# GarciaLnk/LlamaRec

Measured on AMD Instinct MI355X. Metric: users/sec through retrieve+rerank, higher is better.
Workload: dtype bf16; 1 GPU; beauty two-stage: LRURec(V=12086, L=50, D=64, 2 blocks) top-50 with history mask -> Llama-2-7b (32 layers, bf16, random init) single prefill -> verbalizer over 20 candidates; batching=token budget 32768 per step (llamarec_amd/packing.py), rmsnorm_folded_into_gemm=False, llama_layers=32, parallelism=dp1, collective_backend=nccl

## Files before the change

include/llamarec_mi355x.h:

```cpp
#ifndef LLAMAREC_MI355X_H
#define LLAMAREC_MI355X_H

#include <stddef.h>
#include <stdint.h>

#ifdef __cplusplus
extern "C" {
#endif

#define LR_OK 0
#define LR_EINVAL (-1)
#define LR_EUNSUPPORTED (-2)
#define LR_EHIP (-3)
#define LR_EWORKSPACE (-4)

#define LR_MAX_LRU_BLOCKS 4
#define LR_MAX_TOPK 64

const char* lr_last_error(void);
const char* lr_version(void);


typedef struct LrLruBlockWeights {
  const float* params_log;
// ... 110 lines not shown
typedef struct LrRopeScaling {
  int32_t kind;
  float factor, low_freq_factor, high_freq_factor;
  int32_t original_max_positions;
  int32_t reserved[3];
} LrRopeScaling;
int lr_llama_set_rope_scaling(lr_llama_t* h, const LrRopeScaling* s);

typedef struct LrGemma2Ext {
  float attn_softcap;
  float final_softcap;
  float attn_scale;
  int32_t reserved[5];
  const uint16_t* const* attn_out_norm;
  const uint16_t* const* mlp_out_norm;
} LrGemma2Ext;
int lr_llama_set_gemma2(lr_llama_t* h, const LrGemma2Ext* ext);

int lr_llama_set_qkv_bias(lr_llama_t* h, const uint16_t* const* bqkv);

int lr_fold_norm_bf16(const uint16_t* w, const uint16_t* norm_w, int32_t rows, int32_t cols, uint16_t* out,
                      void* hip_stream);
int lr_llama_set_folded_norms(lr_llama_t* h, const uint16_t* const* wqkv_folded, const uint16_t* const* wgu_folded);

int lr_llama_set_last_layer_pruning(lr_llama_t* h, int32_t enable);

size_t lr_llama_workspace_bytes(const lr_llama_t* h, int32_t max_tokens, int32_t max_seqs);

int lr_llama_prefill_verbalize(lr_llama_t* h, const int32_t* packed_ids, const int32_t* cu_seqlens,
                               const int32_t* cu_seqlens_host, int32_t B,
                               const int32_t* label_token_ids, int32_t C, float* out_scores,
                               void* workspace, size_t workspace_bytes, void* hip_stream);

int lr_llama_prefill_verbalize_prefix(lr_llama_t* h, const int32_t* packed_ids, const int32_t* cu_seqlens,
                                      const int32_t* cu_seqlens_host, int32_t B, int32_t prefix_len,
                                      const int32_t* label_token_ids, int32_t C, float* out_scores,
                                      void* workspace, size_t workspace_bytes, void* hip_stream);
int32_t lr_common_prefix_len(const int32_t* packed_ids_host, const int32_t* cu_seqlens_host, int32_t B);

int lr_llama_last_logits(lr_llama_t* h, const int32_t* packed_ids, const int32_t* cu_seqlens,
                         const int32_t* cu_seqlens_host, int32_t B, float* out_logits,
                         void* workspace, size_t workspace_bytes, void* hip_stream);

int lr_llama_pack_qkv(const uint16_t* q, const uint16_t* k, const uint16_t* v, int32_t num_heads,
                      int32_t num_kv_heads, int32_t head_dim, int32_t hidden, uint16_t* out);

// ... 174 lines not shown
```

llamarec_amd/_lib.py:

```python
from __future__ import annotations

import ctypes as C
import os

from . import _abi as A

_HERE = os.path.dirname(os.path.abspath(__file__))
LIB_PATH = os.environ.get("LLAMAREC_LIB") or os.path.join(_HERE, "lib", "libllamarec_mi355x.so")
_lib = None


class LlamaRecError(RuntimeError):
    pass


PROTOTYPES = {
    "lr_last_error": (C.c_char_p, []),
    "lr_version": (C.c_char_p, []),
    "lr_lru_packed_bytes": (C.c_size_t, [C.c_int32, C.c_int32]),
    "lr_lru_pack": (C.c_int, [C.POINTER(A.LrLruWeightsDesc), C.c_void_p, C.c_size_t]),
    "lr_lru_create": (C.c_int, [C.c_void_p, C.c_size_t, C.c_int32, C.c_int32, C.POINTER(C.c_void_p)]),
    "lr_lru_destroy": (None, [C.c_void_p]),
    "lr_lru_set_encoder_pipeline": (C.c_int, [C.c_void_p, C.c_int32]),
    "lr_lru_workspace_bytes": (C.c_size_t, [C.c_void_p, C.c_int32, C.c_int32, C.c_int32]),
# ... 33 lines not shown
    "lr_lru_train_destroy": (None, [C.c_void_p]),
    "lr_lru_train_workspace_bytes": (C.c_size_t, [C.c_void_p, C.c_int32, C.c_int32]),
    "lr_lru_train_loss_grad": (C.c_int, [C.c_void_p, C.c_void_p, C.c_void_p, C.c_int32, C.c_int32, C.c_void_p,
                                         C.c_void_p, C.c_size_t, C.c_void_p]),
    "lr_lru_train_apply": (C.c_int, [C.c_void_p, C.c_float, C.c_float, C.c_void_p, C.c_void_p]),
    "lr_lru_train_set_graph": (C.c_int, [C.c_void_p, C.c_int32]),
    "lr_lru_train_set_fused": (C.c_int, [C.c_void_p, C.c_int32]),
    "lr_lru_train_set_deterministic": (C.c_int, [C.c_void_p, C.c_int32]),
    "lr_lru_train_buffers": (C.c_int, [C.c_void_p, C.POINTER(C.c_void_p), C.POINTER(C.c_void_p),
                                       C.POINTER(C.c_size_t)]),
    "lr_lru_train_param_range": (C.c_int, [C.c_void_p, C.c_char_p, C.POINTER(C.c_size_t), C.POINTER(C.c_size_t)]),
    "lr_llama_create": (C.c_int, [C.POINTER(A.LrLlamaConfig), C.POINTER(A.LrLlamaWeightsDesc),
                                  C.POINTER(C.c_void_p)]),
    "lr_llama_create_ex": (C.c_int, [C.POINTER(A.LrLlamaConfig), C.POINTER(A.LrLlamaArch), C.POINTER(A.LrLlamaWeightsDesc),
                                     C.POINTER(C.c_void_p)]),
    "lr_llama_destroy": (None, [C.c_void_p]),
    "lr_llama_set_variants": (C.c_int, [C.c_void_p, C.c_int32, C.c_int32]),
    "lr_llama_set_last_layer_pruning": (C.c_int, [C.c_void_p, C.c_int32]),
    "lr_llama_set_rope_scaling": (C.c_int, [C.c_void_p, C.POINTER(A.LrRopeScaling)]),
    "lr_llama_set_gemma2": (C.c_int, [C.c_void_p, C.POINTER(A.LrGemma2Ext)]),
    "lr_llama_set_qkv_bias": (C.c_int, [C.c_void_p, C.c_void_p]),
    "lr_fold_norm_bf16": (C.c_int, [C.c_void_p, C.c_void_p, C.c_int32, C.c_int32, C.c_void_p, C.c_void_p]),
    "lr_llama_set_folded_norms": (C.c_int, [C.c_void_p, C.c_void_p, C.c_void_p]),
    "lr_llama_workspace_bytes": (C.c_size_t, [C.c_void_p, C.c_int32, C.c_int32]),
    "lr_llama_prefill_verbalize": (C.c_int, [C.c_void_p, C.c_void_p, C.c_void_p, C.c_void_p, C.c_int32,
                                             C.c_void_p, C.c_int32, C.c_void_p, C.c_void_p, C.c_size_t,
                                             C.c_void_p]),
    "lr_llama_prefill_verbalize_prefix": (C.c_int, [C.c_void_p, C.c_void_p, C.c_void_p, C.c_void_p, C.c_int32, C.c_int32,
                                                    C.c_void_p, C.c_int32, C.c_void_p, C.c_void_p, C.c_size_t,
                                                    C.c_void_p]),
    "lr_common_prefix_len": (C.c_int32, [C.c_void_p, C.c_void_p, C.c_int32]),
    "lr_llama_last_logits": (C.c_int, [C.c_void_p, C.c_void_p, C.c_void_p, C.c_void_p, C.c_int32,
                                       C.c_void_p, C.c_void_p, C.c_size_t, C.c_void_p]),
    "lr_llama_pack_gate_up": (C.c_int, [C.c_void_p, C.c_void_p, C.c_int32, C.c_int32, C.c_void_p]),
    "lr_llama_pack_qkv": (C.c_int, [C.c_void_p, C.c_void_p, C.c_void_p, C.c_int32, C.c_int32, C.c_int32, C.c_int32,
                                    C.c_void_p]),
    "lr_gemm_bf16_nt": (C.c_int, [C.c_void_p, C.c_void_p, C.c_void_p, C.c_int32, C.c_int32, C.c_int32,
                                  C.c_int32, C.c_void_p]),
    "lr_gemm_bf16_nt_ws": (C.c_int, [C.c_void_p, C.c_void_p, C.c_void_p, C.c_int32, C.c_int32, C.c_int32,
                                     C.c_int32, C.c_void_p, C.c_size_t, C.c_void_p]),
    "lr_attention_varlen": (C.c_int, [C.c_void_p, C.c_void_p, C.c_void_p, C.c_void_p, C.c_int32, C.c_int32,
                                      C.c_int32, C.c_int32, C.c_int32, C.c_void_p]),
    "lr_attention_workspace_bytes": (C.c_size_t, [C.c_int32, C.c_int32, C.c_int32]),
    "lr_attention_varlen_ws": (C.c_int, [C.c_void_p, C.c_void_p, C.c_void_p, C.c_void_p, C.c_void_p, C.c_int32, C.c_int32,
                                         C.c_int32, C.c_int32, C.c_int32, C.c_void_p, C.c_size_t, C.c_void_p]),
    "lr_attention_varlen_prefix": (C.c_int, [C.c_void_p, C.c_void_p, C.c_void_p, C.c_void_p, C.c_int32, C.c_int32, C.c_int32,
# ... 84 lines not shown
```

llamarec_amd/csrc/api_llama.hip:

```cpp
#include <math.h>
#include <stdlib.h>
#include <string.h>

#include <vector>

#include "llama_kernels.h"

typedef unsigned short u16;

extern "C" int lr_llama_create_ex(const LrLlamaConfig* cfg, const LrLlamaArch* arch, const LrLlamaWeightsDesc* w,
                                  lr_llama_t** out) {
  if (!cfg || !w || !out || !w->layers) LR_FAIL(LR_EINVAL, "lr_llama_create: null argument");
  const LrLlamaArch llama_arch = {0, 0, 1.0f, {0, 0, 0, 0, 0}};
  if (!arch) arch = &llama_arch;
  if (arch->norm_style < 0 || arch->norm_style > 1 || arch->mlp_act < 0 || arch->mlp_act > 1 ||
      !(arch->embed_scale > 0.f) || arch->embed_scale != arch->embed_scale)
    LR_FAIL(LR_EINVAL, "lr_llama_create_ex: arch norm_style=%d mlp_act=%d embed_scale=%g", arch->norm_style, arch->mlp_act,
            (double)arch->embed_scale);
  for (int i = 0; i < 5; ++i)
    if (arch->reserved[i]) LR_FAIL(LR_EINVAL, "lr_llama_create_ex: arch reserved word %d is not zero", i);
  if (cfg->num_layers < 1 || cfg->num_heads < 1 || cfg->num_kv_heads < 1 || cfg->vocab_size < 1)
    LR_FAIL(LR_EINVAL, "lr_llama_create: bad config");
  if (cfg->hidden_size % 8 != 0 || cfg->intermediate_size % 16 != 0)
    LR_FAIL(LR_EUNSUPPORTED, "lr_llama_create: hidden_size %% 8 and intermediate_size %% 16 must be 0");
// ... 21 lines not shown
  LR_CHECK_HIP(hipGetDevice(&h->device));
  *out = h;
  return LR_OK;
}

extern "C" int lr_llama_create(const LrLlamaConfig* cfg, const LrLlamaWeightsDesc* w, lr_llama_t** out) {
  return lr_llama_create_ex(cfg, nullptr, w, out);
}

extern "C" int lr_llama_set_variants(lr_llama_t* h, int32_t gemm_variant, int32_t attention_variant) {
  if (!h || (gemm_variant != 0 && gemm_variant != 1 && gemm_variant != 4 && gemm_variant != 5 && gemm_variant != 6) ||
      attention_variant < 0 || attention_variant > 8)
    LR_FAIL(LR_EINVAL, "lr_llama_set_variants: gemm in {0, 1, 4, 5, 6}, attention in {0, 1, 2, 3, 4, 5, 6, 7, 8}");
  h->gemm_variant = gemm_variant;
  h->attn_variant = attention_variant;
  return LR_OK;
}

extern "C" int lr_llama_set_rope_scaling(lr_llama_t* h, const LrRopeScaling* s) {
  if (!h) LR_FAIL(LR_EINVAL, "lr_llama_set_rope_scaling: null handle");
  LR_RUN(lr_check_rope_scaling(s, "lr_llama_set_rope_scaling"));
  if (s) h->rope_scaling = *s;
  else memset(&h->rope_scaling, 0, sizeof(h->rope_scaling));
  return LR_OK;
}

static bool finite_nonneg(float v) { return v >= 0.f && v < __builtin_inff(); }

extern "C" int lr_llama_set_gemma2(lr_llama_t* h, const LrGemma2Ext* e) {
  if (!h) LR_FAIL(LR_EINVAL, "lr_llama_set_gemma2: null handle");
  const int L = h->cfg.num_layers;
  const uint16_t **an = nullptr, **mn = nullptr;
  float scale = 0.f;
  if (e) {
    if (!finite_nonneg(e->attn_softcap) || !finite_nonneg(e->final_softcap) || !finite_nonneg(e->attn_scale))
      LR_FAIL(LR_EINVAL, "lr_llama_set_gemma2: attn_softcap=%g final_softcap=%g attn_scale=%g (finite and >= 0)",
              (double)e->attn_softcap, (double)e->final_softcap, (double)e->attn_scale);
    for (int i = 0; i < 5; ++i)
      if (e->reserved[i]) LR_FAIL(LR_EINVAL, "lr_llama_set_gemma2: reserved word %d is not zero", i);
    if ((e->attn_out_norm == nullptr) != (e->mlp_out_norm == nullptr))
      LR_FAIL(LR_EINVAL, "lr_llama_set_gemma2: give both out-norm arrays or neither");
    if (e->attn_out_norm)
      for (int l = 0; l < L; ++l)
        if (!e->attn_out_norm[l] || !e->mlp_out_norm[l]) LR_FAIL(LR_EINVAL, "lr_llama_set_gemma2: layer %d has a null out-norm", l);
    if (h->arch.norm_style != 1)
      LR_FAIL(LR_EUNSUPPORTED, "lr_llama_set_gemma2: caps and out-norms need a handle with the Gemma norm (norm_style %d)",
// ... 4 lines not shown
      LR_FAIL(LR_EUNSUPPORTED, "lr_llama_set_gemma2: attn_scale %g without a soft cap (the uncapped kernels scale by "
              "head_dim^-0.5 = %g)", (double)scale, (double)own);
    if (h->wqkv_folded) LR_FAIL(LR_EUNSUPPORTED, "lr_llama_set_gemma2: the handle has folded norms");
    if (e->attn_out_norm) {
      an = (const uint16_t**)malloc(sizeof(void*) * L);
      mn = (const uint16_t**)malloc(sizeof(void*) * L);
      if (!an || !mn) {
        free(an);
        free(mn);
        LR_FAIL(LR_EINVAL, "lr_llama_set_gemma2: out of host memory");
      }
      memcpy(an, e->attn_out_norm, sizeof(void*) * L);
      memcpy(mn, e->mlp_out_norm, sizeof(void*) * L);
    }
  }
  free(h->attn_out_norm);
  free(h->mlp_out_norm);
  h->attn_out_norm = an;
  h->mlp_out_norm = mn;
  h->gemma2 = e ? 1 : 0;
  h->attn_softcap = e ? e->attn_softcap : 0.f;
  h->final_softcap = e ? e->final_softcap : 0.f;
  h->attn_scale = (e && e->attn_softcap > 0.f) ? scale : 0.f;
  return LR_OK;
}

extern "C" int lr_llama_set_qkv_bias(lr_llama_t* h, const uint16_t* const* bqkv) {
  if (!h) LR_FAIL(LR_EINVAL, "lr_llama_set_qkv_bias: null handle");
  const int L = h->cfg.num_layers;
  const uint16_t** own = nullptr;
  if (bqkv) {
    for (int l = 0; l < L; ++l)
      if (!bqkv[l]) LR_FAIL(LR_EINVAL, "lr_llama_set_qkv_bias: layer %d has a null bias", l);
    for (int l = 0; l < L; ++l)
      if ((reinterpret_cast<uintptr_t>(bqkv[l]) & 7) || (h->cfg.num_heads * h->cfg.head_dim) % 4 != 0)
        LR_FAIL(LR_EINVAL, "lr_llama_set_qkv_bias: layer %d's bias is not 8-byte aligned", l);
    if (h->wqkv_folded) LR_FAIL(LR_EUNSUPPORTED, "lr_llama_set_qkv_bias: the handle has folded norms");
    own = (const uint16_t**)malloc(sizeof(void*) * L);
    if (!own) LR_FAIL(LR_EINVAL, "lr_llama_set_qkv_bias: out of host memory");
    memcpy(own, bqkv, sizeof(void*) * L);
  }
  free(h->bqkv);
  h->bqkv = own;
  return LR_OK;
}

extern "C" int lr_llama_set_last_layer_pruning(lr_llama_t* h, int32_t enable) {
  if (!h) LR_FAIL(LR_EINVAL, "lr_llama_set_last_layer_pruning: null handle");
  h->prune_last = enable ? 1 : 0;
  return LR_OK;
}

extern "C" void lr_llama_destroy(lr_llama_t* h) {
  if (!h) return;
  free(h->layers);
  free(h->wqkv_folded);
  free(h->wgu_folded);
  free(h->attn_out_norm);
  free(h->mlp_out_norm);
  free(h->bqkv);
  free(h);
}

extern "C" int lr_fold_norm_bf16(const uint16_t* w, const uint16_t* norm_w, int32_t rows, int32_t cols, uint16_t* out,
                                 void* hip_stream) {
  if (!w || !norm_w || !out || rows < 1 || cols < 8) LR_FAIL(LR_EINVAL, "lr_fold_norm_bf16: bad argument");
// ... 2 lines not shown

extern "C" int lr_llama_set_folded_norms(lr_llama_t* h, const uint16_t* const* wqkv_folded,
                                         const uint16_t* const* wgu_folded) {
  if (!h) LR_FAIL(LR_EINVAL, "lr_llama_set_folded_norms: null handle");
  if ((h->arch.norm_style != 0 || h->arch.mlp_act != 0) && (wqkv_folded || wgu_folded))
    LR_FAIL(LR_EUNSUPPORTED, "lr_llama_set_folded_norms: Llama arch only (a Gemma norm (1 + w) cannot be folded into bf16 "
            "weights at HF's rounding, and the GeGLU epilogue takes no row scale)");
  if (h->gemma2 && (wqkv_folded || wgu_folded))
    LR_FAIL(LR_EUNSUPPORTED, "lr_llama_set_folded_norms: not with a Gemma-2 extension (lr_llama_set_gemma2)");
  if (h->bqkv && (wqkv_folded || wgu_folded))
    LR_FAIL(LR_EUNSUPPORTED, "lr_llama_set_folded_norms: not with q/k/v biases (lr_llama_set_qkv_bias)");
  free(h->wqkv_folded);
  free(h->wgu_folded);
  h->wqkv_folded = h->wgu_folded = nullptr;
  if (!wqkv_folded && !wgu_folded) return LR_OK;
  if (!wqkv_folded || !wgu_folded) LR_FAIL(LR_EINVAL, "lr_llama_set_folded_norms: give both arrays or neither");
  const int L = h->cfg.num_layers;
  for (int l = 0; l < L; ++l)
    if (!wqkv_folded[l] || !wgu_folded[l]) LR_FAIL(LR_EINVAL, "lr_llama_set_folded_norms: layer %d has a null matrix", l);
  h->wqkv_folded = (const uint16_t**)malloc(sizeof(void*) * L);
  h->wgu_folded = (const uint16_t**)malloc(sizeof(void*) * L);
  memcpy(h->wqkv_folded, wqkv_folded, sizeof(void*) * L);
  memcpy(h->wgu_folded, wgu_folded, sizeof(void*) * L);
  return LR_OK;
}

struct LlamaWs {
  int32_t *tok_pos, *tok_src, *last_rows, *last_pos, *seg_start;
  float *rope, *rstd;
  u16 *x, *xn, *qkv, *att, *hmid;
  u16 *x_last, *xn_last, *att_last, *h_last, *q_last;
  LrGemmSplitK splitk;
  unsigned* rope16;
  int32_t* prefix_bad;
  void* attn_items;
  size_t attn_items_bytes;
  bool compact;
  size_t total;
};

static LlamaWs carve(const LrLlamaConfig& c, int max_tokens, int max_seqs, char* base) {
  LlamaWs w;
  w.compact = false;
  size_t o = 0;
  auto take = [&](size_t bytes) {
    size_t at = o;
// ... 95 lines not shown
  struct LayerRows { u16 *att, *x, *xn, *hmid; int M, gemm_variant; };
  const LayerRows full = {ws.att, ws.x, ws.xn, ws.hmid, n, gv}, last = {ws.att_last, ws.x_last, ws.xn_last, ws.h_last, B, pv};
  auto rope = [&](const int32_t* tok_pos, int rot_cols) {
    return LrGemmRope{.tok_pos = tok_pos, .cs = ws.rope, .cs16 = ws.rope16, .head_dim = hd, .rot_cols = rot_cols};
  };
  LR_RUN(lr_launch_token_meta(cu, B, P, ws.seg_start, ws.tok_pos, ws.tok_src, ws.last_rows, st, ws.last_pos, ids,
                              ws.prefix_bad));
  LR_RUN(lr_launch_rope_table(ws.rope, plan.maxT, hd, c.rope_theta, st, ws.rope16, &h->rope_scaling));
  if (attn_kernel == LR_ATTN_ROWS256)
    LR_RUN(lr_launch_attn256_items(ws.seg_start, S, n, nh, P, ws.attn_items, ws.attn_items_bytes, st));
  LR_RUN(lr_launch_embed(ids, ws.tok_src, h->embed, c.vocab_size, d, ws.x, n, st, h->arch.embed_scale));
  bool input_normed = false;
#ifdef LR_EXPERIMENTS
  static const bool exp_rstd_once = getenv("LR_EXP_RSTD_ONCE") && getenv("LR_EXP_RSTD_ONCE")[0] == '1';
#define EXP_SKIP_SWEEP (exp_rstd_once && l > 0)
#else
#define EXP_SKIP_SWEEP false
#endif
  for (int l = 0; l < c.num_layers; ++l) {
    const LrLlamaLayerWeights& w = h->layers[l];
    const bool folded = h->wqkv_folded != nullptr;
    const bool last_pruned = l == c.num_layers - 1 && h->prune_last;
    const bool last_q_only = last_pruned && !folded && lr_attention_has_last_row_mode(attn_kernel, hd) && gv != 1;
    if (folded && !EXP_SKIP_SWEEP) LR_RUN(lr_launch_rms_rstd(ws.x, ws.rstd, n, d, c.rms_eps, st));
    if (!folded && !input_normed) LR_RUN(lr_launch_rmsnorm(ws.x, w.input_norm, ws.xn, n, d, c.rms_eps, nullptr, st, ns));
    const int q_w = nh * hd, kv_w = 2 * nkv * hd;
    const u16* const bias = h->bqkv ? h->bqkv[l] : nullptr;
    if (last_q_only) {
      LR_RUN(lr_launch_gemm({.A = ws.xn, .B = w.wqkv + (size_t)q_w * d, .C = ws.qkv, .M = n, .N = kv_w, .K = d,
                             .epi = LR_EPI_ROPE, .variant = gv, .rope = rope(ws.tok_pos, kv_w / 2), .bias = bias ? bias + q_w : nullptr,
                             .splitk = ws.splitk}, st));
      LR_RUN(lr_launch_gather_rows(ws.xn, ws.last_rows, B, d, ws.xn_last, st));
      LR_RUN(lr_launch_gemm({.A = ws.xn_last, .B = w.wqkv, .C = ws.q_last, .M = B, .N = q_w, .K = d, .epi = LR_EPI_ROPE,
                             .variant = pv, .rope = rope(ws.last_pos, q_w), .bias = bias, .splitk = ws.splitk}, st));
      LR_RUN(lr_launch_attention_last(ws.qkv, ws.q_last, ws.att_last, attn.cu, attn.cu_host, S, n, nh, nkv, hd, st, P, a_scale,
                                      a_cap));
    } else {
      LR_RUN(lr_launch_gemm({.A = folded ? ws.x : ws.xn, .B = folded ? h->wqkv_folded[l] : w.wqkv, .C = ws.qkv, .M = n,
                             .N = q_w + kv_w, .K = d, .epi = LR_EPI_ROPE, .variant = gv, .rope = rope(ws.tok_pos, q_w + kv_w / 2),
                             .row_scale = folded ? ws.rstd : nullptr, .bias = bias, .splitk = ws.splitk}, st));
    }
    if (!last_pruned) {
      LR_RUN(lr_launch_attention(attn, attn_kernel, st));
    } else {
      if (!last_q_only && attn_mfma) {
        LR_RUN(lr_launch_attention(attn, attn_kernel, st));
        LR_RUN(lr_launch_gather_rows(ws.att, ws.last_rows, B, nh * hd, ws.att_last, st));
      } else if (!last_q_only) {
        LR_RUN(lr_launch_attention_rows(ws.qkv, ws.att_last, cu, B, ws.last_rows, B, nh, nkv, hd, st, a_scale, a_cap));
      }
      LR_RUN(lr_launch_gather_rows(ws.x, ws.last_rows, B, d, ws.x_last, st));
// ... 360 lines not shown
```

llamarec_amd/csrc/llama_gemm.hip:

```cpp
#include <stdlib.h>

#include "llama_kernels.h"
#include "lr_profile.h"

typedef unsigned short u16;
typedef __bf16 bf16x8 __attribute__((ext_vector_type(8)));
typedef float floatx4 __attribute__((ext_vector_type(4)));
typedef float floatx16 __attribute__((ext_vector_type(16)));
typedef u16 u16x4 __attribute__((ext_vector_type(4)));
typedef u16 u16x8 __attribute__((ext_vector_type(8)));

struct RopeArgs {
  const int32_t* tok_pos;
  const float* cs;
  int head_dim;
  int rot_cols;
  const float* row_scale;
  const unsigned* cs16;
};

template <int EPI, int FOLD = -1, bool BIAS = false>
__device__ __forceinline__ u16x4 epi_value4(floatx4 v, floatx4 up, u16x4 r, const RopeArgs& rope, int row, int col,
                                            const float* pre_rs, const int* pre_pos, const float4* pre_cs = nullptr,
                                            floatx4 bv = floatx4{0.f, 0.f, 0.f, 0.f}) {
// ... 571 lines not shown
    const size_t i = ((size_t)blockIdx.x * 256 + threadIdx.x) * 4;
    if (i >= (size_t)M * n_out) return;
    const int row = (int)(i / n_out), c = (int)(i % n_out);
    const size_t g_off = (size_t)row * N + (c >> 4) * 32 + (c & 15);
    floatx4 g = *reinterpret_cast<const floatx4*>(part + g_off);
    floatx4 u = *reinterpret_cast<const floatx4*>(part + g_off + 16);
    for (int s = 1; s < S; ++s) {
      g += *reinterpret_cast<const floatx4*>(part + s * plane + g_off);
      u += *reinterpret_cast<const floatx4*>(part + s * plane + g_off + 16);
    }
    epi_store4<EPI>(g, u, C, R, (size_t)row * n_out + c, rope, row, c);
  } else {
    const size_t off = ((size_t)blockIdx.x * 256 + threadIdx.x) * 4;
    if (off >= plane) return;
    floatx4 v = *reinterpret_cast<const floatx4*>(part + off);
    for (int s = 1; s < S; ++s) v += *reinterpret_cast<const floatx4*>(part + s * plane + off);
    const int col = (int)(off % N);
    floatx4 bv = floatx4{0.f, 0.f, 0.f, 0.f};
    if (BIAS) bv = bias4(bias_of(bias_arg...), col);
    epi_store4<EPI, BIAS>(v, v, C, R, off, rope, (int)(off / N), col, nullptr, nullptr, bv);
  }
}

static int splitk_factor(int M, int N, int K) {
  const int tiles = ((M + 255) / 256) * (N / 256);
  if (tiles > 128) return 1;
  int S = 256 / tiles;
  if (S > 8) S = 8;
  int min_tiles = 16;
  if (const char* e = getenv("LR_GEMM_SPLITK_MIN_TILES")) {
    const int v = atoi(e);
    if (v >= 1 && v < 16) min_tiles = v;
  }
  const int by_k = (K >> 6) / min_tiles;
  if (S > by_k) S = by_k;
  return S < 2 ? 1 : S;
}

static int gemm256_group_m(int K) {
  static int g = -1;
  if (g < 0) {
    const char* e = getenv("LR_GEMM_GROUP_M");
    g = e ? atoi(e) : 0;
    if (g < 0) g = 0;
  }
  return g ? g : (K >= 8192 ? 4 : G2_GROUP_M);
// ... 158 lines not shown
```

llamarec_amd/csrc/llama_kernels.h:

```cpp
#ifndef LLAMA_KERNELS_H
#define LLAMA_KERNELS_H

#include "lr_common.h"
#include "lr_profile.h"

__device__ __forceinline__ float bf2f(unsigned short b) {
  return __builtin_bit_cast(float, (unsigned int)b << 16);
}
__device__ __forceinline__ unsigned short f2bf(float f) {
  return __builtin_bit_cast(unsigned short, (__bf16)f);
}
__device__ __forceinline__ unsigned short swiglu_bf16(float g, float u) {
  float s = bf2f(f2bf(g * __builtin_amdgcn_rcpf(1.0f + __expf(-g))));
  return f2bf(s * u);
}

__device__ __forceinline__ unsigned short geglu_bf16(float g, float u) {
  const float t = tanhf(0.7978845608028654f * (g + 0.044715f * g * g * g));
  float s = bf2f(f2bf(0.5f * g * (1.0f + t)));
  return f2bf(s * u);
}
template <int NS>
__device__ __forceinline__ unsigned short rms_apply(unsigned short w, unsigned short x, float rstd) {
  if (NS == 0) return f2bf(bf2f(w) * bf2f(f2bf(bf2f(x) * rstd)));
// ... 44 lines not shown
  int head_dim = 0, rot_cols = 0;
};
struct LrGemmSplitK { float* ws = nullptr; size_t bytes = 0; };
struct LrGemmThenNorm {
  const unsigned short* w = nullptr;
  unsigned short* out = nullptr;
  float eps = 0.f;
  int style = 0;
  bool* done = nullptr;
};
struct LrGemmArgs {
  const unsigned short *A, *B;
  unsigned short* C;
  const unsigned short* R = nullptr;
  int M, N, K;
  int epi = LR_EPI_STORE, variant = 0;
  LrGemmRope rope;
  const float* row_scale = nullptr;
  const unsigned short* bias = nullptr;
  LrGemmSplitK splitk;
  LrGemmThenNorm then_norm;
};
int lr_launch_gemm(const LrGemmArgs& g, hipStream_t st);
bool lr_reduce_residual_rmsnorm_fits(int N);
int lr_launch_reduce_residual_rmsnorm(const float* part, int S, unsigned short* C, const unsigned short* R, int M, int N,
                                      const unsigned short* norm_w, unsigned short* norm_out, float eps, hipStream_t st,
                                      int norm_style = 0);
int lr_launch_rms_rstd(const unsigned short* x, float* rstd, int rows, int d, float eps, hipStream_t st);
int lr_launch_fold_norm(const unsigned short* w, const unsigned short* norm_w, unsigned short* out, size_t rows, int cols,
                        hipStream_t st);

static inline int lr_check_segments(const int32_t* cu_host, int S, const char* who, int* shortest = nullptr,
                                    int* longest = nullptr) {
  if (!cu_host || S < 1) LR_FAIL(LR_EINVAL, "%s: %d segments", who, S);
  if (cu_host[0] != 0) LR_FAIL(LR_EINVAL, "%s: cu_seqlens[0] = %d (must be 0)", who, cu_host[0]);
  int lo = 0x7fffffff, hi = 0;
  for (int b = 0; b < S; ++b) {
    const int t = cu_host[b + 1] - cu_host[b];
    if (t < 1) LR_FAIL(LR_EINVAL, "%s: segment %d is empty or negative (cu_seqlens %d -> %d)", who, b, cu_host[b], cu_host[b + 1]);
    lo = t < lo ? t : lo;
    hi = t > hi ? t : hi;
  }
  if (shortest) *shortest = lo;
  if (longest) *longest = hi;
  return LR_OK;
}
// ... 153 lines not shown
```

llamarec_amd/csrc/lr_common.h:

```cpp
#ifndef LR_COMMON_H
#define LR_COMMON_H

#include <hip/hip_runtime.h>
#include <stddef.h>
#include <stdint.h>

#include "../../include/llamarec_mi355x.h"
#include "lr_math.h"
#include "lru_topk_plan.h"

void lr_set_error(const char* fmt, ...);
#define LR_FAIL(code, ...)      \
  do {                          \
    lr_set_error(__VA_ARGS__);  \
    return (code);              \
  } while (0)
#define LR_CHECK_HIP(expr)                                                             \
  do {                                                                                 \
    hipError_t e_ = (expr);                                                            \
    if (e_ != hipSuccess) LR_FAIL(LR_EHIP, "%s: %s", #expr, hipGetErrorString(e_));    \
  } while (0)
#define LR_CHECK_LAUNCH(name)                                                          \
  do {                                                                                 \
    hipError_t e_ = hipGetLastError();                                                 \
// ... 105 lines not shown
                        size_t ws_bytes, hipStream_t st);
int lr_launch_item_scores(const lr_lru* h, const float* q, const int64_t* ids, int B, int L,
                          int exclude_history, float* out_scores, hipStream_t st);

struct lr_llama {
  LrLlamaConfig cfg;
  LrLlamaArch arch;
  const uint16_t* embed;
  const uint16_t* final_norm;
  const uint16_t* lm_head;
  LrLlamaLayerWeights* layers;
  int device;
  int gemm_variant;
  int attn_variant;
  int prune_last;
  const uint16_t** wqkv_folded;
  const uint16_t** wgu_folded;
  LrRopeScaling rope_scaling;
  int gemma2;
  float attn_softcap, final_softcap, attn_scale;
  const uint16_t** attn_out_norm;
  const uint16_t** mlp_out_norm;
  const uint16_t** bqkv;
};

#endif
```

llamarec_amd/csrc/lr_profile.h:

```cpp
#ifndef LR_PROFILE_H
#define LR_PROFILE_H
#include <hip/hip_runtime.h>

#define LR_PROF_GEMM256 0
#define LR_PROF_GEMM_GENERIC 1
#define LR_PROF_ATTN_MFMA 2
#define LR_PROF_ATTN_GENERIC 3
#define LR_PROF_LRU_ENCODE 4
#define LR_PROF_ITEM_TOPK 5
#define LR_PROF_ELEMENTWISE 6

#define LR_PROF_GEMM_TAG(epi, N, K) (((long long)(epi) << 56) | ((long long)(N) << 28) | (long long)(K))
bool lr_prof_begin(int kind, double work, hipStream_t st, long long tag = 0);
void lr_prof_end(hipStream_t st);

struct LrProfScope {
  hipStream_t st;
  bool on;
  LrProfScope(int kind, double work, hipStream_t s, long long tag = 0) : st(s), on(lr_prof_begin(kind, work, s, tag)) {}
  ~LrProfScope() {
    if (on) lr_prof_end(st);
  }
};
#endif
```

llamarec_amd/llm.py:

```python
from __future__ import annotations

import ctypes as C
import json
import os
import re
from dataclasses import dataclass

import numpy as np
import torch

from . import _abi as A
from ._lib import check, lib, stream_ptr

LLAMA2_7B = dict(vocab_size=32000, hidden_size=4096, intermediate_size=11008, num_hidden_layers=32,
                 num_attention_heads=32, num_key_value_heads=32, max_position_embeddings=4096,
                 rms_norm_eps=1e-5, rope_theta=10000.0)
LLAMA3_ROPE_SCALING = dict(rope_type="llama3", factor=32.0, low_freq_factor=1.0, high_freq_factor=4.0,
                           original_max_position_embeddings=8192)
LLAMA32_1B = dict(model_type="llama", vocab_size=128256, hidden_size=2048, intermediate_size=8192, num_hidden_layers=16,
                  num_attention_heads=32, num_key_value_heads=8, head_dim=64, max_position_embeddings=131072,
                  rms_norm_eps=1e-5, rope_theta=500000.0, tie_word_embeddings=True, rope_scaling=dict(LLAMA3_ROPE_SCALING))
LLAMA32_3B = dict(LLAMA32_1B, hidden_size=3072, num_hidden_layers=28, num_attention_heads=24, head_dim=128)
LLAMA31_8B = dict(LLAMA32_1B, hidden_size=4096, intermediate_size=14336, num_hidden_layers=32, num_attention_heads=32,
                  head_dim=128, tie_word_embeddings=False, rope_scaling=dict(LLAMA3_ROPE_SCALING, factor=8.0))
# ... 263 lines not shown
        if v.ndim != 2 or v.shape[0 if m.group(4) == "A" else 1] != r:
            raise ValueError(f"adapter tensor {k!r} has shape {v.shape}: rank {r} expected")
        w[name] = v
    for name in w:
        other = name.replace("lora_A", "lora_B") if "lora_A" in name else name.replace("lora_B", "lora_A")
        if other not in w:
            raise ValueError(f"adapter tensor {name!r} has no partner {other!r}")
    return w


def load_peft_adapter(adapter_path):
    from safetensors import safe_open

    r, alpha, modules = check_adapter_config(json.load(open(os.path.join(adapter_path, "adapter_config.json"))))
    t = {}
    with safe_open(os.path.join(adapter_path, "adapter_model.safetensors"), framework="pt", device="cpu") as f:
        for k in f.keys():
            t[k] = f.get_tensor(k).float().numpy()
    return dict(r=r, alpha=alpha, weights=adapter_weights(t, r, modules), target_modules=modules)


class LlamaRanker:

    def __init__(self, config: dict, device="cuda:0"):
        self.config = dict(config)
        self.device = torch.device(device)
        c = self.config
        self.family = model_family(c)
        self.rope_theta, self.rope_scaling = rope_parameters(c)
        self.hd = c.get("head_dim") or c["hidden_size"] // c["num_attention_heads"]
        windowed = (c.get("model_type") == "mistral" or self.family in ("gemma2", "phi3")
                    or (self.family == "qwen2" and c["use_sliding_window"]))
        self.max_prompt_len = c.get("sliding_window") if windowed else None
        self._window_owner = {"gemma2": "Gemma-2", "phi3": "Phi-3", "qwen2": "Qwen2"}.get(self.family, "Mistral")
        self._h = C.c_void_p()
        self._tensors = {}
        self._ws = None
        self._layers_arr = None
        self._folded_arr = None
        self.fold_norms = False
        self.training = False
        self.default_gemm_variant = 6 if self.family == "qwen2" else 0

    @classmethod
    def from_state_dict(cls, state_dict, config, device="cuda:0", lora=None, nf4=False):
        self = cls(config, device)
        dev = self.device
        scratch = {}

        def nf4_roundtrip(w):
            w = w.to(torch.bfloat16).contiguous()
            need = lib().lr_nf4_scratch_bytes(w.numel())
            if scratch.get("n", 0) < need:
                scratch["buf"], scratch["n"] = torch.empty(need, dtype=torch.uint8, device=dev), need
            with torch.cuda.device(dev):
                check(lib().lr_nf4_roundtrip_bf16(w.data_ptr(), w.numel(), 1, w.data_ptr(), scratch["buf"].data_ptr(),
                                                  scratch["n"], stream_ptr()), "lr_nf4_roundtrip_bf16")
            return w

        def t(name):
            w = state_dict[name]
            if not isinstance(w, torch.Tensor):
# ... 157 lines not shown
        desc = A.LrLlamaWeightsDesc(embed=T["embed"].data_ptr(), final_norm=T["final_norm"].data_ptr(),
                                    lm_head=T["lm_head"].data_ptr(), layers=arr)
        h = C.c_void_p()
        with torch.cuda.device(self.device):
            torch.cuda.synchronize()
            check(lib().lr_llama_create_ex(C.byref(cfg), C.byref(self.arch()), C.byref(desc), C.byref(h)), "lr_llama_create_ex")
        self._h, self._layers_arr = h, arr
        if self.rope_scaling is not None:
            rs = self.rope_scaling
            words = A.LrRopeScaling(kind=1, factor=float(rs["factor"]), low_freq_factor=float(rs["low_freq_factor"]),
                                    high_freq_factor=float(rs["high_freq_factor"]),
                                    original_max_positions=int(rs["original_max_position_embeddings"]))
            check(lib().lr_llama_set_rope_scaling(self._h, C.byref(words)), "lr_llama_set_rope_scaling")
        if self.family == "gemma2":
            ext, self._gemma2_arrs = self.gemma2_ext()
            check(lib().lr_llama_set_gemma2(self._h, C.byref(ext)), "lr_llama_set_gemma2")
        if "0.bqkv" in T:
            self._bqkv_arr = (C.c_void_p * L)(*[T[f"{i}.bqkv"].data_ptr() for i in range(L)])
            check(lib().lr_llama_set_qkv_bias(self._h, self._bqkv_arr), "lr_llama_set_qkv_bias")
        if self.default_gemm_variant:
            self.set_variants(gemm=self.default_gemm_variant)
        if self.fold_norms:
            self.set_fold_norms(True)

    def gemma2_ext(self):
        c, T, L = self.config, self._tensors, self.config["num_hidden_layers"]
        ext = A.LrGemma2Ext(attn_softcap=float(c["attn_logit_softcapping"] or 0.0),
                            final_softcap=float(c["final_logit_softcapping"] or 0.0),
                            attn_scale=float(c["query_pre_attn_scalar"]) ** -0.5)
        arrs = None
        if "0.attn_out_norm" in T:
            arrs = ((C.c_void_p * L)(*[T[f"{i}.attn_out_norm"].data_ptr() for i in range(L)]),
                    (C.c_void_p * L)(*[T[f"{i}.mlp_out_norm"].data_ptr() for i in range(L)]))
            ext.attn_out_norm, ext.mlp_out_norm = arrs
        return ext, arrs

    def set_fold_norms(self, enable=True):
        T, L = self._tensors, self.config["num_hidden_layers"]
        if enable and self.family in ("gemma", "gemma2"):
            raise NotImplementedError("folded norms: Gemma's (1 + w) RMSNorm cannot be folded into bf16 weights at HF's rounding")
        if enable and self.family == "qwen2":
            raise NotImplementedError("folded norms: not with Qwen2's q/k/v biases (lr_llama_set_qkv_bias)")
        if not enable:
            check(lib().lr_llama_set_folded_norms(self._h, None, None), "lr_llama_set_folded_norms")
            for i in range(L):
                T.pop(f"{i}.wqkv_folded", None)
                T.pop(f"{i}.wgu_folded", None)
            self._folded_arr = None
            self.fold_norms = False
            return self
        qa, ga = (C.c_void_p * L)(), (C.c_void_p * L)()
        with torch.cuda.device(self.device):
            for i in range(L):
                for name, norm, arr in (("wqkv", "input_norm", qa), ("wgu", "post_norm", ga)):
                    w = T[f"{i}.{name}"]
                    out = torch.empty_like(w)
                    check(lib().lr_fold_norm_bf16(w.data_ptr(), T[f"{i}.{norm}"].data_ptr(), w.shape[0], w.shape[1],
                                                  out.data_ptr(), stream_ptr()), "lr_fold_norm_bf16")
                    T[f"{i}.{name}_folded"] = out
                    arr[i] = out.data_ptr()
            torch.cuda.synchronize()
            check(lib().lr_llama_set_folded_norms(self._h, qa, ga), "lr_llama_set_folded_norms")
        self._folded_arr = (qa, ga)
        self.fold_norms = True
        return self

    def set_variants(self, gemm=0, attention=0):
        check(lib().lr_llama_set_variants(self._h, gemm, attention), "lr_llama_set_variants")
        return self

    def set_last_layer_pruning(self, enable=True):
        check(lib().lr_llama_set_last_layer_pruning(self._h, int(bool(enable))), "lr_llama_set_last_layer_pruning")
        return self

    def eval(self):
        return self

    def __del__(self):
        try:
            if self._h.value:
                lib().lr_llama_destroy(self._h)
        except Exception:
            pass

    def _check_lengths(self, cu_host):
        if self.max_prompt_len is not None and int(np.diff(cu_host).max()) > self.max_prompt_len:
            raise NotImplementedError(f"a prompt of {int(np.diff(cu_host).max())} tokens exceeds {self._window_owner}'s sliding window of "
# ... 52 lines not shown
```

llamarec_amd/rank_train.py:

```python
from __future__ import annotations

import ctypes as C
import json
import math
import os
import re
import shutil

import numpy as np
import torch

from . import _abi as A
from ._lib import check, lib, stream_ptr
from .llm import LORA_MODULE_BLOCK, LlamaRanker, expand_target_modules, pack_prompts

IGNORE = -100
PEFT_KEY = "base_model.model.model.layers.{l}.{block}.{p}_proj.lora_{ab}.weight"
DEFAULT_TARGET_MODULES = ("q_proj", "v_proj")


def peft_key(layer, module, ab):
    return PEFT_KEY.format(l=layer, block=LORA_MODULE_BLOCK[module], p=module[:-len("_proj")], ab=ab)


# ... 287 lines not shown
            w.copy_((w.float() + delta).to(torch.bfloat16))

        for l in range(self.L):
            def delta(mod):
                return s * (p[f"layers.{l}.{mod}.lora_B"] @ p[f"layers.{l}.{mod}.lora_A"])

            w = rk._tensors[f"{l}.wqkv"]
            for mod in self.target_modules:
                if mod == "q_proj":
                    add_(w[:nq], rk._interleave_rope_rows(delta(mod)))
                elif mod == "k_proj":
                    add_(w[nq:nq + nkv], rk._interleave_rope_rows(delta(mod)))
                elif mod == "v_proj":
                    add_(w[nq + nkv:], delta(mod))
                elif mod == "o_proj":
                    add_(rk._tensors[f"{l}.wo"], delta(mod))
                elif mod == "down_proj":
                    add_(rk._tensors[f"{l}.wdown"], delta(mod))
                else:
                    gu = rk._tensors[f"{l}.wgu"].view(f // 16, 2, 16, -1)
                    add_(gu[:, 0 if mod == "gate_proj" else 1], delta(mod).view(f // 16, 16, -1))
        if rk.fold_norms:
            rk.set_fold_norms(True)
        self.merged = True
        return rk

    def __del__(self):
        try:
            if self._h.value:
                lib().lr_llama_lora_destroy(self._h)
        except Exception:
            pass


class LLMTrainSamples:

    def __init__(self, args, u2seq, text_dict, tokenizer, prompter=None, rng=None):
        from . import prompt as P

        self.P, self.args = P, args
        self.max_len = getattr(args, "llm_max_history", P.LLM_MAX_HISTORY)
        self.num_items = args.num_items
        self.neg = getattr(args, "llm_negative_sample_size", 19)
        self.rng = rng if rng is not None else np.random
        self.text_dict, self.tokenizer = text_dict, tokenizer
        self.prompter = prompter or P.Prompter()
# ... 291 lines not shown
```

Baseline: 156.0 users/s.

## Precompute layer-0 QKV per vocab token and gather instead of GEMM

Layer 0's input is just the token embedding, so its rmsnorm plus QKV projection (bias included) depends only on the token id. This builds a vocab-by-QKV-width bf16 table once at weight load. In prefill, layer 0's rmsnorm and QKV GEMM are replaced by a row gather with fused RoPE. The aim is to remove one large GEMM per step, at the cost of roughly 0.8 GB of device memory (under the 1 GB cap) and a memory-bound gather of 24 KB per token. The table is rebuilt whenever weights, bias, fold settings or LoRA merges change.

New measurement: 157.2 users/s (median of 6 runs). No clear change (+0.8%).

```diff
diff --git a/include/llamarec_mi355x.h b/include/llamarec_mi355x.h
--- a/include/llamarec_mi355x.h
+++ b/include/llamarec_mi355x.h
@@ -156,6 +156,11 @@
 int lr_fold_norm_bf16(const uint16_t* w, const uint16_t* norm_w, int32_t rows, int32_t cols, uint16_t* out,
                       void* hip_stream);
 int lr_llama_set_folded_norms(lr_llama_t* h, const uint16_t* const* wqkv_folded, const uint16_t* const* wgu_folded);
+
+size_t lr_llama_qkv0_table_bytes(const lr_llama_t* h);
+size_t lr_llama_qkv0_build_workspace_bytes(const lr_llama_t* h);
+int lr_llama_qkv0_build(lr_llama_t* h, uint16_t* table, void* workspace, size_t workspace_bytes, void* hip_stream);
+int lr_llama_set_qkv0_table(lr_llama_t* h, const uint16_t* table);
 
 int lr_llama_set_last_layer_pruning(lr_llama_t* h, int32_t enable);
 
diff --git a/llamarec_amd/_lib.py b/llamarec_amd/_lib.py
--- a/llamarec_amd/_lib.py
+++ b/llamarec_amd/_lib.py
@@ -79,6 +79,10 @@
     "lr_llama_set_qkv_bias": (C.c_int, [C.c_void_p, C.c_void_p]),
     "lr_fold_norm_bf16": (C.c_int, [C.c_void_p, C.c_void_p, C.c_int32, C.c_int32, C.c_void_p, C.c_void_p]),
     "lr_llama_set_folded_norms": (C.c_int, [C.c_void_p, C.c_void_p, C.c_void_p]),
+    "lr_llama_qkv0_table_bytes": (C.c_size_t, [C.c_void_p]),
+    "lr_llama_qkv0_build_workspace_bytes": (C.c_size_t, [C.c_void_p]),
+    "lr_llama_qkv0_build": (C.c_int, [C.c_void_p, C.c_void_p, C.c_void_p, C.c_size_t, C.c_void_p]),
+    "lr_llama_set_qkv0_table": (C.c_int, [C.c_void_p, C.c_void_p]),
     "lr_llama_workspace_bytes": (C.c_size_t, [C.c_void_p, C.c_int32, C.c_int32]),
     "lr_llama_prefill_verbalize": (C.c_int, [C.c_void_p, C.c_void_p, C.c_void_p, C.c_void_p, C.c_int32,
                                              C.c_void_p, C.c_int32, C.c_void_p, C.c_void_p, C.c_size_t,
diff --git a/llamarec_amd/csrc/api_llama.hip b/llamarec_amd/csrc/api_llama.hip
--- a/llamarec_amd/csrc/api_llama.hip
+++ b/llamarec_amd/csrc/api_llama.hip
@@ -67,6 +67,7 @@
   LR_RUN(lr_check_rope_scaling(s, "lr_llama_set_rope_scaling"));
   if (s) h->rope_scaling = *s;
   else memset(&h->rope_scaling, 0, sizeof(h->rope_scaling));
+  h->qkv0_table = nullptr;
   return LR_OK;
 }
 
@@ -117,6 +118,7 @@
   h->attn_softcap = e ? e->attn_softcap : 0.f;
   h->final_softcap = e ? e->final_softcap : 0.f;
   h->attn_scale = (e && e->attn_softcap > 0.f) ? scale : 0.f;
+  h->qkv0_table = nullptr;
   return LR_OK;
 }
 
@@ -137,6 +139,7 @@
   }
   free(h->bqkv);
   h->bqkv = own;
+  h->qkv0_table = nullptr;
   return LR_OK;
 }
 
@@ -185,6 +188,76 @@
   h->wgu_folded = (const uint16_t**)malloc(sizeof(void*) * L);
   memcpy(h->wqkv_folded, wqkv_folded, sizeof(void*) * L);
   memcpy(h->wgu_folded, wgu_folded, sizeof(void*) * L);
+  h->qkv0_table = nullptr;
+  return LR_OK;
+}
+
+#define LR_QKV0_CHUNK 4096
+
+static size_t qkv0_width(const LrLlamaConfig& c) { return (size_t)(c.num_heads + 2 * c.num_kv_heads) * c.head_dim; }
+
+struct Qkv0BuildWs {
+  int32_t* ids;
+  u16 *x, *xn;
+  size_t total;
+};
+static Qkv0BuildWs qkv0_carve(const LrLlamaConfig& c, char* base) {
+  Qkv0BuildWs w;
+  const size_t chunk = c.vocab_size < LR_QKV0_CHUNK ? c.vocab_size : LR_QKV0_CHUNK;
+  size_t o = 0;
+  auto take = [&](size_t bytes) {
+    size_t at = o;
+    o += lr_align_up(bytes, 256);
+    return base + at;
+  };
+  w.ids = (int32_t*)take((size_t)c.vocab_size * 4);
+  w.x = (u16*)take(chunk * c.hidden_size * 2);
+  w.xn = (u16*)take(chunk * c.hidden_size * 2);
+  w.total = o;
+  return w;
+}
+
+__global__ __launch_bounds__(256) void qkv0_ids_kernel(int32_t* ids, int n) {
+  const int i = blockIdx.x * 256 + threadIdx.x;
+  if (i < n) ids[i] = i;
+}
+
+extern "C" size_t lr_llama_qkv0_table_bytes(const lr_llama_t* h) {
+  return h ? (size_t)h->cfg.vocab_size * qkv0_width(h->cfg) * 2 : 0;
+}
+
+extern "C" size_t lr_llama_qkv0_build_workspace_bytes(const lr_llama_t* h) {
+  return h ? qkv0_carve(h->cfg, nullptr).total : 0;
+}
+
+extern "C" int lr_llama_qkv0_build(lr_llama_t* h, uint16_t* table, void* workspace, size_t workspace_bytes, void* hip_stream) {
+  if (!h) LR_FAIL(LR_EINVAL, "lr_llama_qkv0_build: null handle");
+  if (!table || (reinterpret_cast<uintptr_t>(table) & 15)) LR_FAIL(LR_EINVAL, "lr_llama_qkv0_build: the table is null or not 16-byte aligned");
+  const LrLlamaConfig& c = h->cfg;
+  const Qkv0BuildWs ws = qkv0_carve(c, (char*)workspace);
+  if (!workspace || ws.total > workspace_bytes)
+    LR_FAIL(LR_EWORKSPACE, "lr_llama_qkv0_build: workspace needs %zu bytes, have %zu", ws.total, workspace ? workspace_bytes : (size_t)0);
+  hipStream_t st = (hipStream_t)hip_stream;
+  const int V = c.vocab_size, d = c.hidden_size;
+  const size_t width = qkv0_width(c);
+  const int gv = h->gemm_variant == 5 ? 0 : h->gemm_variant;
+  const LrLlamaLayerWeights& w = h->layers[0];
+  hipLaunchKernelGGL(qkv0_ids_kernel, dim3((V + 255) / 256), dim3(256), 0, st, ws.ids, V);
+  LR_CHECK_LAUNCH("qkv0_ids_kernel");
+  for (int base = 0; base < V; base += LR_QKV0_CHUNK) {
+    const int m = V - base < LR_QKV0_CHUNK ? V - base : LR_QKV0_CHUNK;
+    LR_RUN(lr_launch_embed(ws.ids + base, nullptr, h->embed, V, d, ws.x, m, st, h->arch.embed_scale));
+    LR_RUN(lr_launch_rmsnorm(ws.x, w.input_norm, ws.xn, m, d, c.rms_eps, nullptr, st, h->arch.norm_style));
+    LR_RUN(lr_launch_gemm({.A = ws.xn, .B = w.wqkv, .C = table + (size_t)base * width, .M = m, .N = (int)width, .K = d,
+                           .epi = LR_EPI_STORE, .variant = gv, .bias = h->bqkv ? h->bqkv[0] : nullptr}, st));
+  }
+  return LR_OK;
+}
+
+extern "C" int lr_llama_set_qkv0_table(lr_llama_t* h, const uint16_t* table) {
+  if (!h) LR_FAIL(LR_EINVAL, "lr_llama_set_qkv0_table: null handle");
+  if (reinterpret_cast<uintptr_t>(table) & 15) LR_FAIL(LR_EINVAL, "lr_llama_set_qkv0_table: the table is not 16-byte aligned");
+  h->qkv0_table = table;
   return LR_OK;
 }
 
@@ -326,11 +399,15 @@
     const bool folded = h->wqkv_folded != nullptr;
     const bool last_pruned = l == c.num_layers - 1 && h->prune_last;
     const bool last_q_only = last_pruned && !folded && lr_attention_has_last_row_mode(attn_kernel, hd) && gv != 1;
+    const int q_w = nh * hd, kv_w = 2 * nkv * hd;
+    const bool by_table = l == 0 && h->qkv0_table && !folded && !last_pruned && gv != 5;
     if (folded && !EXP_SKIP_SWEEP) LR_RUN(lr_launch_rms_rstd(ws.x, ws.rstd, n, d, c.rms_eps, st));
-    if (!folded && !input_normed) LR_RUN(lr_launch_rmsnorm(ws.x, w.input_norm, ws.xn, n, d, c.rms_eps, nullptr, st, ns));
-    const int q_w = nh * hd, kv_w = 2 * nkv * hd;
+    if (!folded && !input_normed && !by_table) LR_RUN(lr_launch_rmsnorm(ws.x, w.input_norm, ws.xn, n, d, c.rms_eps, nullptr, st, ns));
     const u16* const bias = h->bqkv ? h->bqkv[l] : nullptr;
-    if (last_q_only) {
+    if (by_table) {
+      LR_RUN(lr_launch_qkv0_lookup(ids, ws.tok_src, h->qkv0_table, c.vocab_size, q_w + kv_w, ws.qkv, n,
+                                   rope(ws.tok_pos, q_w + kv_w / 2), st));
+    } else if (last_q_only) {
       LR_RUN(lr_launch_gemm({.A = ws.xn, .B = w.wqkv + (size_t)q_w * d, .C = ws.qkv, .M = n, .N = kv_w, .K = d,
                              .epi = LR_EPI_ROPE, .variant = gv, .rope = rope(ws.tok_pos, kv_w / 2), .bias = bias ? bias + q_w : nullptr,
                              .splitk = ws.splitk}, st));
diff --git a/llamarec_amd/csrc/llama_gemm.hip b/llamarec_amd/csrc/llama_gemm.hip
--- a/llamarec_amd/csrc/llama_gemm.hip
+++ b/llamarec_amd/csrc/llama_gemm.hip
@@ -617,6 +617,51 @@
   }
 }
 
+template <int PIECE>
+__global__ __launch_bounds__(256) void qkv0_lookup_kernel(const int32_t* __restrict__ ids, const int32_t* __restrict__ tok_src,
+                                                          const u16* __restrict__ table, int vocab, int width,
+                                                          u16* __restrict__ out, RopeArgs rope) {
+  typedef u16 u16xp __attribute__((ext_vector_type(PIECE)));
+  const int row = blockIdx.x;
+  int id = ids[tok_src ? tok_src[row] : row];
+  if (id < 0 || id >= vocab) id = 0;
+  const int pos = rope.tok_pos[row];
+  const u16* src = table + (size_t)id * width;
+  u16* dst = out + (size_t)row * width;
+  for (int c = threadIdx.x * PIECE; c < width; c += 256 * PIECE) {
+    u16xp e = *reinterpret_cast<const u16xp*>(src + c);
+#pragma unroll
+    for (int q = 0; q < PIECE; q += 4) {
+      if (c + q >= rope.rot_cols) continue;
+      const floatx4 v = floatx4{bf2f(e[q]), bf2f(e[q + 1]), bf2f(e[q + 2]), bf2f(e[q + 3])};
+      const u16x4 o = epi_value4<LR_EPI_ROPE, 0, false>(v, v, u16x4{0, 0, 0, 0}, rope, row, c + q, nullptr, &pos);
+#pragma unroll
+      for (int j = 0; j < 4; ++j) e[q + j] = o[j];
+    }
+    *reinterpret_cast<u16xp*>(dst + c) = e;
+  }
+}
+
+int lr_launch_qkv0_lookup(const int32_t* ids, const int32_t* tok_src, const u16* table, int vocab, int width, u16* out, int n,
+                          const LrGemmRope& r, hipStream_t st) {
+  if (n <= 0) return LR_OK;
+  if (!ids || !table || !out || vocab < 1 || width < 4 || width % 4 != 0)
+    LR_FAIL(LR_EINVAL, "qkv0 lookup: bad arguments (vocab=%d width=%d)", vocab, width);
+  if (!r.tok_pos || !r.cs || r.head_dim < 2 || r.head_dim % 4 != 0 || r.rot_cols % 4 != 0 || r.rot_cols < 0 || r.rot_cols > width)
+    LR_FAIL(LR_EINVAL, "qkv0 lookup: bad rope arguments (head_dim=%d rot_cols=%d)", r.head_dim, r.rot_cols);
+  const bool wide = width % 8 == 0 && (reinterpret_cast<uintptr_t>(table) & 15) == 0 && (reinterpret_cast<uintptr_t>(out) & 15) == 0;
+  if (!wide && ((reinterpret_cast<uintptr_t>(table) & 7) || (reinterpret_cast<uintptr_t>(out) & 7)))
+    LR_FAIL(LR_EINVAL, "qkv0 lookup: table and output must be 8-byte aligned");
+  const RopeArgs rope{r.tok_pos, r.cs, r.head_dim, r.rot_cols, nullptr, r.cs16};
+  LrProfScope prof(LR_PROF_QKV0_LOOKUP, 2.0 * n * (double)width * 2, st);
+  if (wide)
+    hipLaunchKernelGGL(qkv0_lookup_kernel<8>, dim3((unsigned)n), dim3(256), 0, st, ids, tok_src, table, vocab, width, out, rope);
+  else
+    hipLaunchKernelGGL(qkv0_lookup_kernel<4>, dim3((unsigned)n), dim3(256), 0, st, ids, tok_src, table, vocab, width, out, rope);
+  LR_CHECK_LAUNCH("qkv0_lookup_kernel");
+  return LR_OK;
+}
+
 static int splitk_factor(int M, int N, int K) {
   const int tiles = ((M + 255) / 256) * (N / 256);
   if (tiles > 128) return 1;
diff --git a/llamarec_amd/csrc/llama_kernels.h b/llamarec_amd/csrc/llama_kernels.h
--- a/llamarec_amd/csrc/llama_kernels.h
+++ b/llamarec_amd/csrc/llama_kernels.h
@@ -90,6 +90,8 @@
   LrGemmThenNorm then_norm;
 };
 int lr_launch_gemm(const LrGemmArgs& g, hipStream_t st);
+int lr_launch_qkv0_lookup(const int32_t* ids, const int32_t* tok_src, const unsigned short* table, int vocab, int width,
+                          unsigned short* out, int n, const LrGemmRope& rope, hipStream_t st);
 bool lr_reduce_residual_rmsnorm_fits(int N);
 int lr_launch_reduce_residual_rmsnorm(const float* part, int S, unsigned short* C, const unsigned short* R, int M, int N,
                                       const unsigned short* norm_w, unsigned short* norm_out, float eps, hipStream_t st,
diff --git a/llamarec_amd/csrc/lr_common.h b/llamarec_amd/csrc/lr_common.h
--- a/llamarec_amd/csrc/lr_common.h
+++ b/llamarec_amd/csrc/lr_common.h
@@ -151,6 +151,7 @@
   const uint16_t** attn_out_norm;
   const uint16_t** mlp_out_norm;
   const uint16_t** bqkv;
+  const uint16_t* qkv0_table;
 };
 
 #endif
diff --git a/llamarec_amd/csrc/lr_profile.h b/llamarec_amd/csrc/lr_profile.h
--- a/llamarec_amd/csrc/lr_profile.h
+++ b/llamarec_amd/csrc/lr_profile.h
@@ -9,6 +9,7 @@
 #define LR_PROF_LRU_ENCODE 4
 #define LR_PROF_ITEM_TOPK 5
 #define LR_PROF_ELEMENTWISE 6
+#define LR_PROF_QKV0_LOOKUP 7
 
 #define LR_PROF_GEMM_TAG(epi, N, K) (((long long)(epi) << 56) | ((long long)(N) << 28) | (long long)(K))
 bool lr_prof_begin(int kind, double work, hipStream_t st, long long tag = 0);
diff --git a/llamarec_amd/llm.py b/llamarec_amd/llm.py
--- a/llamarec_amd/llm.py
+++ b/llamarec_amd/llm.py
@@ -309,6 +309,9 @@
 
 class LlamaRanker:
 
+    qkv0_table_max_bytes = 1 << 30
+    qkv0_table_min_hidden = 1024
+
     def __init__(self, config: dict, device="cuda:0"):
         self.config = dict(config)
         self.device = torch.device(device)
@@ -325,6 +328,8 @@
         self._ws = None
         self._layers_arr = None
         self._folded_arr = None
+        self._qkv0_table = None
+        self.qkv0_table = None
         self.fold_norms = False
         self.training = False
         self.default_gemm_variant = 6 if self.family == "qwen2" else 0
@@ -528,6 +533,32 @@
             self.set_variants(gemm=self.default_gemm_variant)
         if self.fold_norms:
             self.set_fold_norms(True)
+        self._refresh_qkv0_table()
+
+    @property
+    def has_qkv0_table(self):
+        return self._qkv0_table is not None
+
+    def _refresh_qkv0_table(self):
+        L_ = lib()
+        check(L_.lr_llama_set_qkv0_table(self._h, None), "lr_llama_set_qkv0_table")
+        self._qkv0_table = None
+        need = L_.lr_llama_qkv0_table_bytes(self._h)
+        wanted = self.config["hidden_size"] >= self.qkv0_table_min_hidden if self.qkv0_table is None else self.qkv0_table
+        if not wanted or self.fold_norms or need == 0 or need > self.qkv0_table_max_bytes:
+            return
+        with torch.cuda.device(self.device):
+            table = torch.empty(need // 2, dtype=torch.bfloat16, device=self.device)
+            ws = torch.empty(L_.lr_llama_qkv0_build_workspace_bytes(self._h), dtype=torch.uint8, device=self.device)
+            check(L_.lr_llama_qkv0_build(self._h, table.data_ptr(), ws.data_ptr(), ws.numel(), stream_ptr()), "lr_llama_qkv0_build")
+            torch.cuda.synchronize()
+            check(L_.lr_llama_set_qkv0_table(self._h, table.data_ptr()), "lr_llama_set_qkv0_table")
+        self._qkv0_table = table
+
+    def set_qkv0_table(self, enable=True):
+        self.qkv0_table = None if enable is None else bool(enable)
+        self._refresh_qkv0_table()
+        return self
 
     def gemma2_ext(self):
         c, T, L = self.config, self._tensors, self.config["num_hidden_layers"]
@@ -554,6 +585,7 @@
                 T.pop(f"{i}.wgu_folded", None)
             self._folded_arr = None
             self.fold_norms = False
+            self._refresh_qkv0_table()
             return self
         qa, ga = (C.c_void_p * L)(), (C.c_void_p * L)()
         with torch.cuda.device(self.device):
@@ -569,6 +601,7 @@
             check(lib().lr_llama_set_folded_norms(self._h, qa, ga), "lr_llama_set_folded_norms")
         self._folded_arr = (qa, ga)
         self.fold_norms = True
+        self._refresh_qkv0_table()
         return self
 
     def set_variants(self, gemm=0, attention=0):
diff --git a/llamarec_amd/rank_train.py b/llamarec_amd/rank_train.py
--- a/llamarec_amd/rank_train.py
+++ b/llamarec_amd/rank_train.py
@@ -333,6 +333,7 @@
                     add_(gu[:, 0 if mod == "gate_proj" else 1], delta(mod).view(f // 16, 16, -1))
         if rk.fold_norms:
             rk.set_fold_norms(True)
+        rk._refresh_qkv0_table()
         self.merged = True
         return rk
 
```
